# snphbaum/scikit-gpuppy

Hardware: NVIDIA B200
Metric: fit_s_per_iter (lower is better)
Workload: dtype f64

## Files before the change

### scikit-gpuppy_b200/csrc/gpk.cu

```cuda
#include "../../include/gpk.h"
#include "../../include/gpk_test.h"

#include <climits>
#include <new>
#include <vector>

#include "dgemm_dmma.cuh"
#include "factor.cuh"
#include "se_kernels.cuh"
#include "exact_kernels.cuh"
#include "periodic_kernels.cuh"

namespace gpk {
thread_local char g_err[512] = {0};
thread_local long g_launch_count = 0;
thread_local bool g_prof_on = false;
static thread_local std::vector<ProfPair> g_prof;
void prof_push(cudaEvent_t a, cudaEvent_t b) { g_prof.push_back(ProfPair{a, b}); }

struct Handle {
  int n = 0, d = 0, npad = 0;
  double *X = nullptr, *W = nullptr;
  bool own_X = false, own_W = false;
  double *x = nullptr, *xT = nullptr, *t = nullptr, *y = nullptr, *alpha = nullptr, *dL = nullptr;
  double* scal = nullptr;
  int* info = nullptr;
  double* part = nullptr; size_t part_elems = 0;
  double* G = nullptr; size_t G_elems = 0;
  double* colsq = nullptr; size_t colsq_elems = 0;
  double* pairdot = nullptr;
  double* dots = nullptr; size_t dots_elems = 0;
  long batch_rows = 0;
  SEHyper hyp;
  int kind = KIND_SE;
  double theta[3 * MAX_D + 2];
  bool factored = false, have_inverse = false;
  bool matrix_state = false;
  double logdet = 0.0, quad = 0.0, alpha2 = 0.0;
  cudaStream_t st = nullptr;
  cudaStream_t side = nullptr;
  std::vector<cudaEvent_t> events;
  int ev_next = 0;
  bool oz_want = false;
  bool oz_on = false;
  int oz_moduli_req = 0;
  size_t oz_out_cap = 0;
  oz::Workspace oz;
  oz::Workspace ozq;
  oz::Operand xs;
  bool x_sliced = false;
  cudaStream_t chain_st = nullptr;
  std::vector<cudaStream_t> ovl_st;
  std::vector<oz::Workspace> ovl_ws;
  cudaEvent_t ev_in = nullptr, ev_out = nullptr;
  bool ovl_on = false;
  double* raw_pinned = nullptr;
  bool grad_pending = false;
};

thread_local int g_overlap_T = 1;

static void release_overlap(Handle* h) {
  for (auto& w : h->ovl_ws) w.release();
  h->ovl_ws.clear();
  for (auto& s : h->ovl_st) if (s) { cudaStreamSynchronize(s); cudaStreamDestroy(s); }
  h->ovl_st.clear();
  if (h->chain_st) { cudaStreamSynchronize(h->chain_st); cudaStreamDestroy(h->chain_st); h->chain_st = nullptr; }
  if (h->ev_in) { cudaEventDestroy(h->ev_in); h->ev_in = nullptr; }
  if (h->ev_out) { cudaEventDestroy(h->ev_out); h->ev_out = nullptr; }
  h->ovl_on = false;
}

static int ensure_overlap(Handle* h) {
  if (h->ovl_on || !h->oz_on || !g_overlap_T) return 0;
  int depths = 0;
  size_t need = 0;
  for (long hh = h->npad / 2 / TILE * TILE; hh >= h->oz.min_dim; hh = hh / 2 / TILE * TILE) {
    need += (size_t)h->oz.S * (hh + TILE) * (3 * (hh + TILE) + round_up_l(hh + TILE, 256)) + 6 * hh * sizeof(double);
    ++depths;
  }
  if (depths == 0) return 0;
  size_t free_b = 0, total_b = 0;
  if (cudaMemGetInfo(&free_b, &total_b) != cudaSuccess) { cudaGetLastError(); return 0; }
  if (free_b < need + ((size_t)28 << 30)) return 0;
  int least = 0, greatest = 0;
  GPK_CUDA_OK(cudaDeviceGetStreamPriorityRange(&least, &greatest));
  GPK_CUDA_OK(cudaStreamCreateWithPriority(&h->chain_st, cudaStreamNonBlocking, greatest));
  GPK_CUDA_OK(cudaEventCreateWithFlags(&h->ev_in, cudaEventDisableTiming));
  GPK_CUDA_OK(cudaEventCreateWithFlags(&h->ev_out, cudaEventDisableTiming));
  h->ovl_st.assign(depths, nullptr);
// ... 40 lines not shown
    }
  }
  return 0;
}

static int ensure(double** p, size_t* have, size_t need) {
  if (*have >= need) return 0;
  if (*p) GPK_CUDA_OK(cudaFree(*p));
  *p = nullptr;
  *have = 0;
  GPK_CUDA_OK(cudaMalloc((void**)p, need * sizeof(double)));
  *have = need;
  return 0;
}

__global__ void __launch_bounds__(256) col_sum_kernel(const double* __restrict__ part, long nrows, int ncols,
                                                      double* __restrict__ out) {
  __shared__ double red[8];
  const int c = blockIdx.x;
  double s = 0.0;
  for (long r = threadIdx.x; r < nrows; r += 256) s += part[r * ncols + c];
  s = block_sum_256(s, red);
  if (threadIdx.x == 0) out[c] = s;
}

__global__ void set_int_kernel(int* p, int v) { *p = v; }
__global__ void __launch_bounds__(256) axpy_kernel(double* __restrict__ y, const double* __restrict__ x, int n, double a) {
  const int i = blockIdx.x * 256 + threadIdx.x;
  if (i < n) y[i] = fma(a, x[i], y[i]);
}

static int launch_se_tiles(const double* x1, int n1, const double* x2, int n2, int d, const SEHyper& hyp, double* out,
                           long ld, int rows_out, int cols_out, int add_noise, int pad_identity, int lower_only,
                           cudaStream_t st) {
  SETileArgs a;
  a.x1 = x1; a.n1 = n1; a.x2 = x2; a.n2 = n2; a.d = d;
  a.out = out; a.ld = ld; a.rows_out = rows_out; a.cols_out = cols_out;
  a.add_noise = add_noise; a.pad_identity = pad_identity; a.lower_only = lower_only;
  a.vec_ok = ((ld % 2) == 0 && (reinterpret_cast<uintptr_t>(out) % 16) == 0) ? 1 : 0;
  if (rows_out <= 0 || cols_out <= 0) return 0;
  if (hyp.kind == KIND_PERIODIC) {
    dim3 pgrid((cols_out + PER_T - 1) / PER_T, (rows_out + PER_T - 1) / PER_T);
    periodic_tile_kernel<<<pgrid, 256, 0, st>>>(a, hyp);
    GPK_LAUNCH_OK();
    return 0;
  }
  dim3 grid((cols_out + TILE - 1) / TILE, (rows_out + TILE - 1) / TILE);
  se_tile_kernel<<<grid, SE_THREADS, 0, st>>>(a, hyp);
  GPK_LAUNCH_OK();
  return 0;
}

static int solve_one(Handle* h, const double* b_pad, double* y, double* out) {
  const int npad = h->npad;
  trmv_lower_kernel<<<(npad + 7) / 8, 256, 0, h->st>>>(h->X, npad, npad, b_pad, y);
  GPK_LAUNCH_OK();
  const int nchunks = (npad + TRMVT_ROWS - 1) / TRMVT_ROWS;
  GPK_TRY(ensure(&h->part, &h->part_elems, (size_t)nchunks * npad));
  dim3 grid(npad / 128, nchunks);
  trmv_lower_T_partial_kernel<<<grid, 128, 0, h->st>>>(h->X, npad, npad, y, h->part);
  GPK_LAUNCH_OK();
  sum_chunks_kernel<<<(npad + 255) / 256, 256, 0, h->st>>>(h->part, nchunks, npad, npad, out, 1.0, 0.0);
  GPK_LAUNCH_OK();
  return 0;
}

template <int DP>
static int launch_trace(Handle* h, int d0, int trb, int tre, double* partial) {
  const int nt = h->npad / TILE;
  const size_t smem = (size_t)2 * h->d * (TILE + 2) * sizeof(double);
  GPK_CUDA_OK(cudaFuncSetAttribute(grad_trace_kernel<DP>, cudaFuncAttributeMaxDynamicSharedMemorySize, (int)smem));
  dim3 grid(nt, tre - trb);
  grad_trace_kernel<DP><<<grid, 256, smem, h->st>>>(h->W, h->npad, h->alpha, h->x, h->n, h->d, d0, h->hyp, trb, partial);
  GPK_LAUNCH_OK();
  return 0;
}

static int trace_sums(Handle* h, int trb, int tre, double* raw_host, double* async_dst = nullptr) {
  const int d = h->d;
  const int nt = h->npad / TILE;
  for (int k = 0; k <= (h->kind == KIND_PERIODIC ? 3 * d + 2 : d + 2); ++k) raw_host[k] = 0.0;
  if (tre <= trb) return 0;
  if (h->kind != KIND_PERIODIC) {
    const int r0 = trb * TILE, r1 = (tre * TILE < h->n) ? tre * TILE : h->n;
    diag_sum_kernel<<<1, 256, 0, h->st>>>(h->W, h->npad, h->alpha, r0, r1, h->scal + 4);
    GPK_LAUNCH_OK();
    GPK_CUDA_OK(cudaMemcpyAsync(async_dst ? async_dst : raw_host + d + 1, h->scal + 4, 2 * sizeof(double),
                                cudaMemcpyDeviceToHost, h->st));
  }
  if (h->kind == KIND_PERIODIC) {
    const int DPp = d <= 4 ? 4 : d <= 8 ? 8 : 16;
    const int nc = 3 * DPp + 2;
    const long nsl = (long)nt * (tre - trb);
    GPK_TRY(ensure(&h->part, &h->part_elems, (size_t)nsl * nc + nc));
    double* psums = h->part + (size_t)nsl * nc;
    dim3 pgrid(nt, tre - trb);
    if (DPp == 4) periodic_trace_kernel<4><<<pgrid, 256, 0, h->st>>>(h->W, h->npad, h->alpha, h->x, h->n, d, h->hyp, trb, h->part);
    else if (DPp == 8) periodic_trace_kernel<8><<<pgrid, 256, 0, h->st>>>(h->W, h->npad, h->alpha, h->x, h->n, d, h->hyp, trb, h->part);
    else periodic_trace_kernel<16><<<pgrid, 256, 0, h->st>>>(h->W, h->npad, h->alpha, h->x, h->n, d, h->hyp, trb, h->part);
    GPK_LAUNCH_OK();
    col_sum_kernel<<<nc, 256, 0, h->st>>>(h->part, nsl, nc, psums);
    GPK_LAUNCH_OK();
    double ph[50];
    GPK_CUDA_OK(cudaMemcpyAsync(ph, psums, nc * sizeof(double), cudaMemcpyDeviceToHost, h->st));
    GPK_CUDA_OK(cudaStreamSynchronize(h->st));
    raw_host[0] = ph[0];
    for (int k = 0; k < d; ++k) {
      raw_host[1 + k] = ph[1 + k];
      raw_host[1 + d + k] = ph[1 + DPp + k];
      raw_host[1 + 2 * d + k] = ph[1 + 2 * DPp + k];
    }
    raw_host[3 * d + 1] = ph[3 * DPp + 1];
    raw_host[3 * d + 2] = 0.0;
    return 0;
  }
  int DP = d <= 4 ? 4 : d <= 8 ? 8 : d <= 16 ? 16 : 32;
  const long nslots = (long)nt * (tre - trb);
  const int nchunks = (d + DP - 1) / DP;
  GPK_TRY(ensure(&h->part, &h->part_elems, (size_t)nslots * (DP + 1) + (size_t)nchunks * (DP + 1)));
  double* sums = h->part + (size_t)nslots * (DP + 1);
  double host[2 * 33];
  for (int d0 = 0, ch = 0; d0 < d; d0 += DP, ++ch) {
    switch (DP) {
      case 4: GPK_TRY(launch_trace<4>(h, d0, trb, tre, h->part)); break;
      case 8: GPK_TRY(launch_trace<8>(h, d0, trb, tre, h->part)); break;
      case 16: GPK_TRY(launch_trace<16>(h, d0, trb, tre, h->part)); break;
      default: GPK_TRY(launch_trace<32>(h, d0, trb, tre, h->part)); break;
    }
    col_sum_kernel<<<DP + 1, 256, 0, h->st>>>(h->part, nslots, DP + 1, sums + ch * (DP + 1));
    GPK_LAUNCH_OK();
    double* dst = async_dst ? async_dst + 4 + ch * (DP + 1) : host + ch * 33;
    GPK_CUDA_OK(cudaMemcpyAsync(dst, sums + ch * (DP + 1), (DP + 1) * sizeof(double), cudaMemcpyDeviceToHost, h->st));
  }
  if (async_dst) return 0;
  GPK_CUDA_OK(cudaStreamSynchronize(h->st));
  for (int d0 = 0, ch = 0; d0 < d; d0 += DP, ++ch) {
    if (d0 == 0) raw_host[0] = host[0];
    for (int k = 0; k < DP && d0 + k < d; ++k) raw_host[1 + d0 + k] = host[ch * 33 + 1 + k];
  }
  return 0;
}

static void trace_unpack(const Handle* h, const double* pinned, double* raw_host) {
  const int d = h->d;
  const int DP = d <= 4 ? 4 : d <= 8 ? 8 : d <= 16 ? 16 : 32;
  raw_host[d + 1] = pinned[0];
  raw_host[d + 2] = pinned[1];
  for (int d0 = 0, ch = 0; d0 < d; d0 += DP, ++ch) {
    const double* src = pinned + 4 + ch * (DP + 1);
    if (d0 == 0) raw_host[0] = src[0];
// ... 242 lines not shown
  cudaFree(hh->x); cudaFree(hh->xT); cudaFree(hh->t); cudaFree(hh->y); cudaFree(hh->alpha); cudaFree(hh->dL);
  cudaFree(hh->scal); cudaFree(hh->info);
  for (auto& e : hh->events) if (e) cudaEventDestroy(e);
  if (hh->side) { cudaStreamSynchronize(hh->side); cudaStreamDestroy(hh->side); }
  if (hh->part) cudaFree(hh->part);
  if (hh->G) cudaFree(hh->G);
  if (hh->colsq) cudaFree(hh->colsq);
  if (hh->dots) cudaFree(hh->dots);
  hh->oz.release();
  hh->ozq.release();
  release_overlap(hh);
  if (hh->raw_pinned) cudaFreeHost(hh->raw_pinned);
  delete hh;
  return 0;
}

int gpk_set_stream(gpk_handle h, void* stream) {
  H_OR_FAIL(h);
  hh->st = reinterpret_cast<cudaStream_t>(stream);
  return 0;
}

int gpk_set_kernel(gpk_handle h, int kind) {
  H_OR_FAIL(h);
  if (kind != KIND_SE && kind != KIND_PERIODIC) { snprintf(g_err, sizeof(g_err), "unknown kernel kind %d", kind); return -2; }
  if (kind == KIND_PERIODIC && hh->d > PER_MAX_D) {
    snprintf(g_err, sizeof(g_err), "the periodic covariance supports d <= %d", PER_MAX_D);
    return -2;
  }
  hh->kind = kind;
  hh->factored = false;
  hh->have_inverse = false;
  hh->x_sliced = false;
  return 0;
}

int gpk_kernel_matrix_periodic(const double* x1, int64_t n1, const double* x2, int64_t n2, int64_t d, const double* theta,
                               int noise_mode, double* out, int64_t ld, void* stream) {
  SEHyper hyp;
  GPK_TRY(set_hyper(hyp, theta, (int)d, KIND_PERIODIC));
  return launch_se_tiles(x1, (int)n1, x2, (int)n2, (int)d, hyp, out, ld, (int)n1, (int)n2, noise_mode, 0, 0,
                         reinterpret_cast<cudaStream_t>(stream));
}

int gpk_set_route(gpk_handle h, int int8, int64_t min_dim, int moduli, int64_t plane_cap_bytes) {
  H_OR_FAIL(h);
  if (int8 && (min_dim != 0 && (min_dim < 2 * TILE || min_dim % TILE))) {
    snprintf(g_err, sizeof(g_err), "gpk_set_route: min_dim must be 0 (default 2048) or a multiple of 128 >= 256");
    return -2;
  }
  if (int8 && moduli != 0 && (moduli < oz::CRT_MIN_MODULI || moduli > oz::CRT_MAX_MODULI)) {
    snprintf(g_err, sizeof(g_err), "gpk_set_route: moduli must be 0 (automatic) or in [%d, %d]", oz::CRT_MIN_MODULI,
             oz::CRT_MAX_MODULI);
    return -2;
  }
  if (int8 && hh->npad > 98304) {
    snprintf(g_err, sizeof(g_err), "gpk_set_route: exact int32 accumulation needs npad <= 98304");
    return -2;
  }
  GPK_CUDA_OK(cudaStreamSynchronize(hh->st));
  hh->oz.release();
  hh->ozq.release();
  release_overlap(hh);
  hh->oz_on = false;
  hh->x_sliced = false;
  hh->factored = false;
  hh->have_inverse = false;
  hh->oz.min_dim = (int8 && min_dim) ? (int)min_dim : 2048;
  hh->oz_moduli_req = int8 ? moduli : 0;
  hh->oz_out_cap = plane_cap_bytes > 0 ? (size_t)plane_cap_bytes : 0;
  hh->oz_want = int8 != 0 && hh->npad >= hh->oz.min_dim;
  return 0;
}

int gpk_get_route(gpk_handle h, int* out) {
  H_OR_FAIL(h);
  const int S = hh->oz_on ? hh->oz.S
                          : (hh->oz_moduli_req ? hh->oz_moduli_req : oz::crt_moduli_for(hh->npad, 54));
  out[0] = hh->oz_want ? 1 : 0;
  out[1] = hh->oz_want ? S : 0;
  out[2] = hh->oz.min_dim;
  out[3] = hh->oz_want ? oz::crt_bits(hh->npad, S) : 53;
  return 0;
}

int gpk_set_batch_rows(gpk_handle h, int64_t rows) {
  H_OR_FAIL(h);
  hh->batch_rows = rows < 0 ? 0 : rows;
  return 0;
}

int gpk_set_data(gpk_handle h, const double* x_dev, const double* t_dev) {
  H_OR_FAIL(h);
  GPK_CUDA_OK(cudaMemcpyAsync(hh->x, x_dev, (size_t)hh->n * hh->d * sizeof(double), cudaMemcpyDeviceToDevice, hh->st));
  GPK_CUDA_OK(cudaMemsetAsync(hh->t, 0, (size_t)hh->npad * sizeof(double), hh->st));
  GPK_CUDA_OK(cudaMemcpyAsync(hh->t, t_dev, (size_t)hh->n * sizeof(double), cudaMemcpyDeviceToDevice, hh->st));
  transpose_x_kernel<<<(hh->npad + 255) / 256, 256, 0, hh->st>>>(hh->x, hh->n, hh->d, hh->xT, hh->npad);
  GPK_LAUNCH_OK();
  hh->factored = false;
  hh->have_inverse = false;
  return 0;
}

int gpk_kernel_matrix(const double* x1, int64_t n1, const double* x2, int64_t n2, int64_t d, const double* theta,
                      int add_noise, double* out, int64_t ld, void* stream) {
  SEHyper hyp;
  GPK_TRY(set_hyper(hyp, theta, (int)d));
  return launch_se_tiles(x1, (int)n1, x2, (int)n2, (int)d, hyp, out, ld, (int)n1, (int)n2, add_noise, 0, 0,
                         reinterpret_cast<cudaStream_t>(stream));
}

static int factorize_W(Handle* hh) {
  const int n = hh->n, npad = hh->npad;
  set_int_kernel<<<1, 1, 0, hh->st>>>(hh->info, INT_MAX);
  GPK_LAUNCH_OK();
  FactorCtx c{hh->W, hh->X, (long)npad, hh->dL, hh->info, hh->st};
  hh->ev_next = 0;
  c.side = hh->side; c.ev = hh->events.data(); c.ev_next = &hh->ev_next;
  c.oz = hh->oz_on ? &hh->oz : nullptr;
  const bool ovl = hh->oz_on && hh->ovl_on && g_overlap_T;
  if (ovl) {
    GPK_CUDA_OK(cudaEventRecord(hh->ev_in, hh->st));
    GPK_CUDA_OK(cudaStreamWaitEvent(hh->chain_st, hh->ev_in, 0));
    c.st = hh->chain_st;
    c.ovl_ws = hh->ovl_ws.data(); c.ovl_st = hh->ovl_st.data(); c.ovl_depths = (int)hh->ovl_ws.size();
  }
  const int rc_rec = potrf_inv_node(c, 0, npad);
  if (rc_rec < 0) {
    cudaDeviceSynchronize();
    return rc_rec;
  }
  if (ovl) {
    GPK_CUDA_OK(cudaEventRecord(hh->ev_out, hh->chain_st));
    GPK_CUDA_OK(cudaStreamWaitEvent(hh->st, hh->ev_out, 0));
  }
  GPK_TRY(solve_one(hh, hh->t, hh->y, hh->alpha));
  nll_scalars_kernel<<<1, 256, 0, hh->st>>>(hh->dL, hh->y, hh->alpha, n, hh->scal);
  GPK_LAUNCH_OK();
  int info = 0;
  double sc[3];
  GPK_CUDA_OK(cudaMemcpyAsync(&info, hh->info, sizeof(int), cudaMemcpyDeviceToHost, hh->st));
  GPK_CUDA_OK(cudaMemcpyAsync(sc, hh->scal, 3 * sizeof(double), cudaMemcpyDeviceToHost, hh->st));
  GPK_CUDA_OK(cudaStreamSynchronize(hh->st));
  if (info != INT_MAX) {
    snprintf(g_err, sizeof(g_err), "leading minor %d of K is not positive definite", info);
    return info > 0 ? info : 1;
  }
  hh->logdet = sc[0]; hh->quad = sc[1]; hh->alpha2 = sc[2];
  return 0;
}

int gpk_factorize(gpk_handle h, const double* theta, int want_inverse) {
  H_OR_FAIL(h);
  if (!same_theta(hh, theta)) {
    hh->factored = false;
    hh->have_inverse = false;
    hh->x_sliced = false;
    hh->grad_pending = false;
    GPK_TRY(set_hyper(hh->hyp, theta, hh->d, hh->kind));
    GPK_TRY(ensure_route(hh));
    const int n = hh->n, npad = hh->npad;
    GPK_TRY(launch_se_tiles(hh->x, n, hh->x, n, hh->d, hh->hyp, hh->W, npad, npad, npad,
                            hh->kind == KIND_PERIODIC ? 2 : 1, 1, 1, hh->st));
    const int rc = factorize_W(hh);
    if (rc != 0) return rc;
    memcpy(hh->theta, theta, sizeof(double) * theta_len(hh->kind, hh->d));
    hh->factored = true;
    hh->matrix_state = false;
  }
  if (want_inverse) GPK_TRY(do_lauum(hh));
  return 0;
}

__global__ void __launch_bounds__(256) load_matrix_kernel(const double* __restrict__ K, long ldk, int n,
                                                          double* __restrict__ W, long ld, int npad) {
  const int c = blockIdx.x * 256 + threadIdx.x;
  const int r = blockIdx.y;
  if (c >= npad || (c >> 7) > (r >> 7)) return;
  W[(long)r * ld + c] = (r < n && c < n) ? K[(long)r * ldk + c] : (r == c ? 1.0 : 0.0);
}

int gpk_factorize_matrix(gpk_handle h, const double* K_dev, int64_t ldk, int want_inverse) {
  H_OR_FAIL(h);
  if (!K_dev || ldk < hh->n) { snprintf(g_err, sizeof(g_err), "gpk_factorize_matrix: bad matrix argument"); return -2; }
  hh->factored = false;
  hh->have_inverse = false;
  hh->x_sliced = false;
  GPK_TRY(ensure_route(hh));
  dim3 grid((hh->npad + 255) / 256, hh->npad);
  load_matrix_kernel<<<grid, 256, 0, hh->st>>>(K_dev, ldk, hh->n, hh->W, hh->npad, hh->npad);
  GPK_LAUNCH_OK();
  const int rc = factorize_W(hh);
  if (rc != 0) return rc;
  hh->factored = true;
  hh->matrix_state = true;
  if (want_inverse) GPK_TRY(do_lauum(hh));
  return 0;
}

int gpk_nll_matrix(gpk_handle h, double* nll) {
  H_OR_FAIL(h);
  if (!hh->factored) { snprintf(g_err, sizeof(g_err), "not factored"); return -2; }
  const double two_pi = 6.283185307179586476925286766559;
  *nll = 0.5 * hh->n * log(two_pi) + 0.5 * hh->logdet + 0.5 * hh->quad;
  return 0;
}

int gpk_logdet(gpk_handle h, double* out) {
  H_OR_FAIL(h);
  if (!hh->factored) { snprintf(g_err, sizeof(g_err), "not factored"); return -2; }
  *out = hh->logdet;
  return 0;
}

int gpk_grad_trace_partial(gpk_handle h, int64_t trb, int64_t tre, double* out) {
  H_OR_FAIL(h);
  if (!hh->factored || !hh->have_inverse || hh->matrix_state) { snprintf(g_err, sizeof(g_err), "inverse not available"); return -2; }
  if (hh->kind != KIND_SE) { snprintf(g_err, sizeof(g_err), "sharded trace: Gaussian covariance only"); return -2; }
  const int nt = hh->npad / TILE;
  if (trb < 0) trb = 0;
// ... 117 lines not shown
                            hh->kind == KIND_PERIODIC ? 2 : 0, 0, 0, hh->st));
    rows_dot_kernel<<<(unsigned)((mb + 7) / 8), 256, 0, hh->st>>>(hh->G, npad, (int)mb, npad, hh->alpha, Ka + r0);
    GPK_LAUNCH_OK();
  }
  if (hh->kind != KIND_PERIODIC) {
    axpy_kernel<<<(n + 255) / 256, 256, 0, hh->st>>>(Ka, hh->alpha, n, hh->hyp.vt);
    GPK_LAUNCH_OK();
  }
  residual_max_kernel<<<64, 256, 0, hh->st>>>(Ka, hh->t, hh->alpha, n, mx);
  GPK_LAUNCH_OK();
  unsigned long long bits[3];
  GPK_CUDA_OK(cudaMemcpyAsync(bits, mx, sizeof(bits), cudaMemcpyDeviceToHost, hh->st));
  GPK_CUDA_OK(cudaStreamSynchronize(hh->st));
  for (int i = 0; i < 3; ++i) memcpy(out_host + i, bits + i, sizeof(double));
  return 0;
}

int gpk_get_alpha(gpk_handle h, double* out) {
  H_OR_FAIL(h);
  if (!hh->factored) { snprintf(g_err, sizeof(g_err), "not factored"); return -2; }
  GPK_CUDA_OK(cudaMemcpyAsync(out, hh->alpha, (size_t)hh->n * sizeof(double), cudaMemcpyDeviceToDevice, hh->st));
  return 0;
}

int gpk_import_state(gpk_handle h, const double* theta, const double* alpha_dev, int have_inverse) {
  H_OR_FAIL(h);
  GPK_TRY(set_hyper(hh->hyp, theta, hh->d, hh->kind));
  memcpy(hh->theta, theta, sizeof(double) * theta_len(hh->kind, hh->d));
  GPK_CUDA_OK(cudaMemsetAsync(hh->alpha, 0, (size_t)hh->npad * sizeof(double), hh->st));
  GPK_CUDA_OK(cudaMemcpyAsync(hh->alpha, alpha_dev, (size_t)hh->n * sizeof(double), cudaMemcpyDeviceToDevice, hh->st));
  hh->factored = true;
  hh->matrix_state = false;
  hh->x_sliced = false;
  hh->have_inverse = have_inverse != 0;
  hh->logdet = NAN; hh->quad = NAN; hh->alpha2 = NAN;
  return 0;
}

int gpk_predict(gpk_handle h, const double* xs, int64_t m, double meant, double* mean, double* var, int want_var) {
  H_OR_FAIL(h);
  if (!hh->factored || hh->matrix_state) { snprintf(g_err, sizeof(g_err), "not factored from theta"); return -2; }
  if (m <= 0) return 0;
  const int npad = hh->npad, n = hh->n, d = hh->d;
  const long rows_max = batch_rows_for(hh, m);
  GPK_TRY(ensure_query_ws(hh, rows_max));
  const int nbi = npad / TILE;
  for (int64_t q0 = 0; q0 < m; q0 += rows_max) {
    const long mb = (m - q0) < rows_max ? (long)(m - q0) : rows_max;
    const long rows = round_up_l(mb, TILE);
    GPK_TRY(launch_se_tiles(xs + q0 * d, (int)mb, hh->x, n, d, hh->hyp, hh->G, npad, (int)rows, npad,
                            hh->kind == KIND_PERIODIC ? 2 : 0, 0, 0, hh->st));
    rows_dot_kernel<<<(unsigned)((mb + 7) / 8), 256, 0, hh->st>>>(hh->G, npad, (int)mb, npad, hh->alpha, mean + q0);
    GPK_LAUNCH_OK();
    if (meant != 0.0) {
      add_scalar_kernel<<<(unsigned)((mb + 255) / 256), 256, 0, hh->st>>>(mean + q0, (int)mb, meant);
      GPK_LAUNCH_OK();
    }
    if (want_var) {
      GPK_TRY(quad_forms(hh, rows));
      predict_var_kernel<<<(unsigned)((mb + 255) / 256), 256, 0, hh->st>>>(hh->colsq, rows, nbi, (int)mb,
                                                                            hh->hyp.v + hh->hyp.vt, var + q0);
      GPK_LAUNCH_OK();
    }
  }
  return 0;
}
// ... 242 lines not shown
  if (rc < 0) { cleanup(); return rc; }
  OZ_OK(cudaEventRecord(e1, st));
  if (reps < 1) reps = 1;
  for (int r = 0; r < reps && rc == 0; ++r) rc = oz::gemm_sliced(a, b, C, ldc, alpha, beta, krange, lower_only, st);
  if (rc < 0) { cleanup(); return rc; }
  OZ_OK(cudaEventRecord(e2, st));
  OZ_OK(cudaStreamSynchronize(st));
  if (ms_out) {
    OZ_OK(cudaEventElapsedTime(&ms_out[0], e0, e1));
    OZ_OK(cudaEventElapsedTime(&ms_out[1], e1, e2));
    ms_out[1] /= reps;
  }
#undef OZ_OK
  cleanup();
  return 0;
}

int gpk_test_tune(int group_m, int recon_cw) {
  if (group_m > 0) oz::g_group_m = group_m;
  if (recon_cw == 1 || recon_cw == 2 || recon_cw == 4) oz::g_recon_cw = recon_cw;
  return 0;
}

int gpk_test_position_lock(int on) {
  if (on >= 0 && on <= 2) oz::g_position_lock = on;
  return oz::g_position_lock;
}

int gpk_test_overlap(int on) {
  if (on == 0 || on == 1) g_overlap_T = on;
  return g_overlap_T;
}

int gpk_profile(int on) {
  g_prof_on = on != 0;
  return 0;
}

int gpk_profile_read(double* gemm_ms, int64_t* gemm_launches, int64_t* all_launches, double* max_gemm_ms) {
  double total = 0.0, longest = 0.0;
  for (auto& p : g_prof) {
    float ms = 0.f;
    cudaError_t e = cudaEventSynchronize(p.b);
    if (e == cudaSuccess) e = cudaEventElapsedTime(&ms, p.a, p.b);
    cudaEventDestroy(p.a);
    cudaEventDestroy(p.b);
    if (e != cudaSuccess) {
      snprintf(g_err, sizeof(g_err), "gpk_profile_read: %s", cudaGetErrorString(e));
      g_prof.clear();
      return -1;
    }
    total += ms;
    if (ms > longest) longest = ms;
  }
  if (max_gemm_ms) *max_gemm_ms = longest;
  if (gemm_ms) *gemm_ms = total;
  if (gemm_launches) *gemm_launches = (int64_t)g_prof.size();
  if (all_launches) *all_launches = (int64_t)g_launch_count;
  g_prof.clear();
  g_launch_count = 0;
  return 0;
}

int gpk_microbench_i8(int64_t iters, double seconds, double* out_host) {
  int nsm = 0, dev = 0;
  GPK_CUDA_OK(cudaGetDevice(&dev));
// ... 81 lines not shown
```

### scikit-gpuppy_b200/csrc/se_kernels.cuh

```cuda
#pragma once
#include "gpk_common.cuh"

namespace gpk {

constexpr int MAX_D = 64;
constexpr int SE_DCH = 16;

constexpr int KIND_SE = 0;
constexpr int KIND_PERIODIC = 1;

struct SEHyper {
  double v, vt;
  double w[MAX_D];
  double sw[MAX_D];
  int kind;
  double pf[16];
  double w2[16];
  double pr[16];
};

struct SETileArgs {
  const double* x1; int n1;
  const double* x2; int n2;
  int d;
  double* out; long ld;
  int rows_out, cols_out;
  int add_noise;
  int pad_identity;
  int lower_only;
  int vec_ok;
};

constexpr int SE_THREADS = 512;
__global__ void __launch_bounds__(SE_THREADS, 1) se_tile_kernel(SETileArgs p, SEHyper h) {
  const int bj = blockIdx.x, bi = blockIdx.y;
  if (p.lower_only && bj > bi) return;
  __shared__ __align__(16) double xa[SE_DCH][TILE];
  __shared__ __align__(16) double xb[SE_DCH][TILE];
  const int tid = threadIdx.x;
  const int tx = tid & 15, ty = (tid >> 4) & 15, tz = tid >> 8;
  const int row0 = bi * TILE, col0 = bj * TILE;

  double acc[4][8];
#pragma unroll
  for (int a = 0; a < 4; ++a)
#pragma unroll
    for (int b = 0; b < 8; ++b) acc[a][b] = 0.0;

  for (int k0 = 0; k0 < p.d; k0 += SE_DCH) {
    const int kc = min(SE_DCH, p.d - k0);
    __syncthreads();
    for (int idx = tid; idx < TILE * SE_DCH; idx += SE_THREADS) {
      const int r = idx / SE_DCH, k = idx % SE_DCH;
      double va = 0.0, vb = 0.0;
      if (k < kc) {
        const double s = h.sw[k0 + k];
        if (row0 + r < p.n1) va = p.x1[(long)(row0 + r) * p.d + k0 + k] * s;
        if (col0 + r < p.n2) vb = p.x2[(long)(col0 + r) * p.d + k0 + k] * s;
      }
      xa[k][r] = va;
      xb[k][r] = vb;
    }
    __syncthreads();
    for (int k = 0; k < kc; ++k) {
      double av[4];
      double2 bv[4];
#pragma unroll
      for (int a = 0; a < 4; ++a) av[a] = xa[k][ty + 16 * (a + 4 * tz)];
#pragma unroll
      for (int b = 0; b < 4; ++b) bv[b] = *reinterpret_cast<const double2*>(&xb[k][32 * b + 2 * tx]);
#pragma unroll
      for (int a = 0; a < 4; ++a)
#pragma unroll
        for (int b = 0; b < 4; ++b) {
          const double d0 = av[a] - bv[b].x, d1 = av[a] - bv[b].y;
          acc[a][2 * b] = fma(d0, d0, acc[a][2 * b]);
          acc[a][2 * b + 1] = fma(d1, d1, acc[a][2 * b + 1]);
        }
    }
  }

#pragma unroll
  for (int a = 0; a < 4; ++a) {
    const int row = row0 + ty + 16 * (a + 4 * tz);
    if (row >= p.rows_out) continue;
#pragma unroll
    for (int b = 0; b < 4; ++b) {
      const int col = col0 + 32 * b + 2 * tx;
      double o[2];
#pragma unroll
      for (int e = 0; e < 2; ++e) {
        const int c = col + e;
        double val;
        if (row < p.n1 && c < p.n2) {
          val = h.v * exp(-0.5 * acc[a][2 * b + e]);
          if (p.add_noise && row == c) val += h.vt;
        } else {
          val = (p.pad_identity && row == c) ? 1.0 : 0.0;
        }
        o[e] = val;
      }
      double* dst = p.out + (long)row * p.ld + col;
      if (p.vec_ok && col + 1 < p.cols_out) {
        *reinterpret_cast<double2*>(dst) = make_double2(o[0], o[1]);
      } else {
        if (col < p.cols_out) dst[0] = o[0];
        if (col + 1 < p.cols_out) dst[1] = o[1];
      }
    }
  }
}

template <int DP>
__global__ void __launch_bounds__(256, (DP <= 16) ? 2 : 1)
grad_trace_kernel(const double* __restrict__ Kinv, long ld, const double* __restrict__ alpha,
                  const double* __restrict__ x, int n, int d, int d0 , SEHyper h,
                  int tile_row_begin, double* __restrict__ partial ) {
  const int bj = blockIdx.x, bi = tile_row_begin + blockIdx.y;
  double* out = partial + ((long)blockIdx.y * gridDim.x + blockIdx.x) * (DP + 1);
  if (bj > bi) {
    if (threadIdx.x <= DP) out[threadIdx.x] = 0.0;
    return;
  }

  extern __shared__ __align__(16) double gsm[];
  constexpr int XLD = TILE + 2;
  constexpr int RT = 2;
  double* xa = gsm;
  double* xb = gsm + (long)d * XLD;
  __shared__ double al_a[TILE], al_b[TILE];
  __shared__ double red[8];
  const int tid = threadIdx.x;
  const int row0 = bi * TILE, col0 = bj * TILE;

  for (int idx = tid; idx < TILE * d; idx += 256) {
    const int r = idx / d, k = idx % d;
    xa[k * XLD + r] = (row0 + r < n) ? x[(long)(row0 + r) * d + k] : 0.0;
    xb[k * XLD + r] = (col0 + r < n) ? x[(long)(col0 + r) * d + k] : 0.0;
  }
  if (tid < TILE) {
    al_a[tid] = (row0 + tid < n) ? alpha[row0 + tid] : 0.0;
    al_b[tid] = (col0 + tid < n) ? alpha[col0 + tid] : 0.0;
  }
  __syncthreads();

  double g0 = 0.0;
  double gk[DP];
#pragma unroll
  for (int k = 0; k < DP; ++k) gk[k] = 0.0;

  const int c = tid & 127;
// ... 46 lines not shown
          sq[2 * i2][k] = d0v * d0v;
          sq[2 * i2 + 1][k] = d1v * d1v;
          dist[2 * i2] = fma(wk, sq[2 * i2][k], dist[2 * i2]);
          dist[2 * i2 + 1] = fma(wk, sq[2 * i2 + 1][k], dist[2 * i2 + 1]);
        }
      } else {
#pragma unroll
        for (int i = 0; i < RT; ++i) sq[i][k] = 0.0;
      }
    }
    for (int k = d0 + DP; k < d; ++k) {
      const double bv = xb[k * XLD + c];
#pragma unroll
      for (int i = 0; i < RT; ++i) {
        const double df = xa[k * XLD + r0 + i] - bv;
        dist[i] = fma(h.w[k] * df, df, dist[i]);
      }
    }
#pragma unroll
    for (int i = 0; i < RT; ++i) {
      const double pk = m[i] * h.v * exp(-0.5 * dist[i]);
      g0 += pk;
#pragma unroll
      for (int k = 0; k < DP; ++k) gk[k] = fma(pk, sq[i][k], gk[k]);
    }
  }

  double s = block_sum_256(g0, red);
  if (tid == 0) out[0] = s;
#pragma unroll
  for (int k = 0; k < DP; ++k) {
    s = block_sum_256(gk[k], red);
    if (tid == 0) out[1 + k] = s;
  }
}

__global__ void __launch_bounds__(256) diag_sum_kernel(const double* __restrict__ W, long ld,
                                                       const double* __restrict__ alpha, int r0, int r1,
                                                       double* __restrict__ out) {
  __shared__ double red[8];
  double s = 0.0, a2 = 0.0;
  for (int i = r0 + threadIdx.x; i < r1; i += 256) {
    s += W[(long)i * ld + i];
    a2 = fma(alpha[i], alpha[i], a2);
  }
  s = block_sum_256(s, red);
  a2 = block_sum_256(a2, red);
  if (threadIdx.x == 0) {
    out[0] = s;
    out[1] = a2;
  }
}

struct GAArgs {
  const double* xT; long ldxt;
  int n, npad, d, P;
  const double* U;
  const double* S;
  int sigma_full;
  double* G; long ldg;
  int rows_pad;
  int Q;
};

__global__ void __launch_bounds__(256) ga_build_kernel(GAArgs p, SEHyper h) {
  const int q = blockIdx.y;
// ... 121 lines not shown
```

### scikit-gpuppy_b200/skgpuppy/_native.py

```python
import ctypes
import os

import numpy as np

_HERE = os.path.dirname(os.path.abspath(__file__))
_LIB_PATH = os.path.join(_HERE, "libgpk.so")
_lib = None

c_double_p = ctypes.POINTER(ctypes.c_double)
c_int_p = ctypes.POINTER(ctypes.c_int)
i64 = ctypes.c_int64
vp = ctypes.c_void_p

SIGNATURES = {
    "gpk_version": (ctypes.c_int, []),
    "gpk_last_error": (ctypes.c_char_p, []),
    "gpk_npad": (i64, [i64]),
    "gpk_create": (ctypes.c_int, [i64, i64, vp, vp, ctypes.POINTER(vp)]),
    "gpk_destroy": (ctypes.c_int, [vp]),
    "gpk_set_stream": (ctypes.c_int, [vp, vp]),
    "gpk_set_data": (ctypes.c_int, [vp, vp, vp]),
    "gpk_kernel_matrix": (ctypes.c_int, [vp, i64, vp, i64, i64, c_double_p, ctypes.c_int, vp, i64, vp]),
    "gpk_factorize": (ctypes.c_int, [vp, c_double_p, ctypes.c_int]),
    "gpk_factorize_matrix": (ctypes.c_int, [vp, vp, i64, ctypes.c_int]),
    "gpk_nll_matrix": (ctypes.c_int, [vp, c_double_p]),
    "gpk_logdet": (ctypes.c_int, [vp, c_double_p]),
    "gpk_nll_grad": (ctypes.c_int, [vp, c_double_p, c_double_p, c_double_p, ctypes.c_int]),
    "gpk_grad_trace_partial": (ctypes.c_int, [vp, i64, i64, c_double_p]),
    "gpk_solve": (ctypes.c_int, [vp, vp, i64, vp]),
    "gpk_inverse": (ctypes.c_int, [vp, vp, i64]),
    "gpk_solve_residual": (ctypes.c_int, [vp, c_double_p]),
    "gpk_get_alpha": (ctypes.c_int, [vp, vp]),
    "gpk_import_state": (ctypes.c_int, [vp, c_double_p, vp, ctypes.c_int]),
    "gpk_predict": (ctypes.c_int, [vp, vp, i64, ctypes.c_double, vp, vp, ctypes.c_int]),
    "gpk_predict_cross": (ctypes.c_int, [vp, vp, i64, i64, vp, ctypes.c_double, vp, vp]),
    "gpk_propagate_ga": (ctypes.c_int, [vp, vp, vp, i64, ctypes.c_int, ctypes.c_double, vp, vp]),
    "gpk_propagate_ga_parts": (ctypes.c_int, [vp, vp, vp, i64, ctypes.c_int, vp, vp]),
    "gpk_propagate_exact": (ctypes.c_int, [vp, vp, vp, vp, vp, i64, ctypes.c_double, vp, vp]),
    "gpk_set_kernel": (ctypes.c_int, [vp, ctypes.c_int]),
    "gpk_kernel_matrix_periodic": (ctypes.c_int, [vp, i64, vp, i64, i64, c_double_p, ctypes.c_int, vp, i64, vp]),
    "gpk_set_route": (ctypes.c_int, [vp, ctypes.c_int, i64, ctypes.c_int, i64]),
    "gpk_get_route": (ctypes.c_int, [vp, c_int_p]),
    "gpk_set_batch_rows": (ctypes.c_int, [vp, i64]),
}

TEST_SIGNATURES = {
    "gpk_test_gemm": (ctypes.c_int, [ctypes.c_int, ctypes.c_int, ctypes.c_int, vp, i64, vp, i64, vp, i64, i64, i64,
                                     i64, ctypes.c_double, ctypes.c_double, ctypes.c_int, ctypes.c_int, vp, vp, i64,
                                     vp]),
    "gpk_test_potrf_inv": (ctypes.c_int, [vp, vp, i64, i64, vp, c_int_p, vp]),
    "gpk_test_lauum": (ctypes.c_int, [vp, vp, i64, i64, vp]),
    "gpk_test_oz_residues": (ctypes.c_int, [vp, i64, i64, i64, ctypes.c_int, ctypes.c_int, ctypes.c_int, vp, vp, vp]),
    "gpk_test_oz_gemm": (ctypes.c_int, [vp, i64, ctypes.c_int, ctypes.c_int, vp, i64, ctypes.c_int, ctypes.c_int, vp, i64,
                                        i64, i64, i64, ctypes.c_double, ctypes.c_double, ctypes.c_int, ctypes.c_int,
                                        ctypes.c_int, i64, ctypes.c_int, ctypes.POINTER(ctypes.c_float), vp]),
    "gpk_test_tune": (ctypes.c_int, [ctypes.c_int, ctypes.c_int]),
    "gpk_test_overlap": (ctypes.c_int, [ctypes.c_int]),
    "gpk_test_position_lock": (ctypes.c_int, [ctypes.c_int]),
    "gpk_profile": (ctypes.c_int, [ctypes.c_int]),
    "gpk_profile_read": (ctypes.c_int, [c_double_p, ctypes.POINTER(i64), ctypes.POINTER(i64), c_double_p]),
    "gpk_microbench": (ctypes.c_int, [ctypes.c_int, i64, c_double_p]),
    "gpk_microbench_i8": (ctypes.c_int, [i64, ctypes.c_double, c_double_p]),
}


class GpkError(RuntimeError):
    pass


def lib_path():
    return _LIB_PATH


def load():
    global _lib
    if _lib is not None:
        return _lib
    if not os.path.exists(_LIB_PATH):
        raise GpkError(
            "libgpk.so not found at %s: build it with `python scikit-gpuppy_b200/build_native.py` "
            "(there is no CPU fallback)" % _LIB_PATH)
    lib = ctypes.CDLL(_LIB_PATH)
    for name, (res, args) in list(SIGNATURES.items()) + list(TEST_SIGNATURES.items()):
        fn = getattr(lib, name)
        fn.restype = res
        fn.argtypes = args
    _lib = lib
    return lib


# ... 35 lines not shown
```

Before: 0.2906.

## Mirror SE kernel into upper triangle and read stored K in gradient trace

When building the squared-exponential K for large npad, the tile kernel also writes each lower tile, transposed through shared memory, into the upper triangle of W. The upper triangle then still holds K after the lower triangle is factored and inverted. The gradient trace kernel for off-diagonal tiles can then read the stored K values with a cp.async multi-stage pipeline instead of recomputing the exponentials. Diagonal tiles still use the recomputing kernel. This trades exp recomputation for extra strided global writes during matrix build and extra memory reads during the trace, and it assumes the inverse only overwrites the lower triangle.

```diff
diff --git a/scikit-gpuppy_b200/csrc/gpk.cu b/scikit-gpuppy_b200/csrc/gpk.cu
--- a/scikit-gpuppy_b200/csrc/gpk.cu
+++ b/scikit-gpuppy_b200/csrc/gpk.cu
@@ -56,6 +56,8 @@
   bool ovl_on = false;
   double* raw_pinned = nullptr;
   bool grad_pending = false;
+  bool knl_in_w = false;
+  bool trace_stored_ok = true;
 };
 
 thread_local int g_overlap_T = 1;
@@ -162,11 +164,16 @@
 
 static int launch_se_tiles(const double* x1, int n1, const double* x2, int n2, int d, const SEHyper& hyp, double* out,
                            long ld, int rows_out, int cols_out, int add_noise, int pad_identity, int lower_only,
-                           cudaStream_t st) {
+                           cudaStream_t st, int mirror = 0) {
   SETileArgs a;
   a.x1 = x1; a.n1 = n1; a.x2 = x2; a.n2 = n2; a.d = d;
   a.out = out; a.ld = ld; a.rows_out = rows_out; a.cols_out = cols_out;
   a.add_noise = add_noise; a.pad_identity = pad_identity; a.lower_only = lower_only;
+  a.mirror = mirror;
+  if (mirror && (x1 != x2 || n1 != n2 || rows_out != cols_out || hyp.kind != KIND_SE)) {
+    snprintf(g_err, sizeof(g_err), "launch_se_tiles: the mirror store needs the square Gaussian K");
+    return -2;
+  }
   a.vec_ok = ((ld % 2) == 0 && (reinterpret_cast<uintptr_t>(out) % 16) == 0) ? 1 : 0;
   if (rows_out <= 0 || cols_out <= 0) return 0;
   if (hyp.kind == KIND_PERIODIC) {
@@ -195,12 +202,27 @@
   return 0;
 }
 
+constexpr int TRACE_STORED_MIN_NPAD = 8192;
+
+static bool trace_reads_k(const Handle* h) { return h->knl_in_w && h->trace_stored_ok && h->kind == KIND_SE; }
+
 template <int DP>
 static int launch_trace(Handle* h, int d0, int trb, int tre, double* partial) {
   const int nt = h->npad / TILE;
   const size_t smem = (size_t)2 * h->d * (TILE + 2) * sizeof(double);
+  dim3 grid(nt, tre - trb);
+  if (trace_reads_k(h)) {
+    const size_t ssmem = grad_trace_stored_smem<DP>();
+    GPK_CUDA_OK(cudaFuncSetAttribute(grad_trace_stored_kernel<DP>, cudaFuncAttributeMaxDynamicSharedMemorySize, (int)ssmem));
+    grad_trace_stored_kernel<DP><<<grid, 256, ssmem, h->st>>>(h->W, h->npad, h->alpha, h->x, h->n, h->d, d0, trb, partial);
+    GPK_LAUNCH_OK();
+    GPK_CUDA_OK(cudaFuncSetAttribute(grad_trace_kernel<DP, true>, cudaFuncAttributeMaxDynamicSharedMemorySize, (int)smem));
+    grad_trace_kernel<DP, true><<<dim3(1, tre - trb), 256, smem, h->st>>>(h->W, h->npad, h->alpha, h->x, h->n, h->d, d0,
+                                                                          h->hyp, trb, partial + (size_t)nt * (tre - trb) * (DP + 1));
+    GPK_LAUNCH_OK();
+    return 0;
+  }
   GPK_CUDA_OK(cudaFuncSetAttribute(grad_trace_kernel<DP>, cudaFuncAttributeMaxDynamicSharedMemorySize, (int)smem));
-  dim3 grid(nt, tre - trb);
   grad_trace_kernel<DP><<<grid, 256, smem, h->st>>>(h->W, h->npad, h->alpha, h->x, h->n, h->d, d0, h->hyp, trb, partial);
   GPK_LAUNCH_OK();
   return 0;
@@ -245,7 +267,7 @@
     return 0;
   }
   int DP = d <= 4 ? 4 : d <= 8 ? 8 : d <= 16 ? 16 : 32;
-  const long nslots = (long)nt * (tre - trb);
+  const long nslots = (long)nt * (tre - trb) + (trace_reads_k(h) ? tre - trb : 0);
   const int nchunks = (d + DP - 1) / DP;
   GPK_TRY(ensure(&h->part, &h->part_elems, (size_t)nslots * (DP + 1) + (size_t)nchunks * (DP + 1)));
   double* sums = h->part + (size_t)nslots * (DP + 1);
@@ -554,6 +576,7 @@
   hh->factored = false;
   hh->have_inverse = false;
   hh->x_sliced = false;
+  hh->knl_in_w = false;
   return 0;
 }
 
@@ -588,6 +611,7 @@
   hh->x_sliced = false;
   hh->factored = false;
   hh->have_inverse = false;
+  hh->knl_in_w = false;
   hh->oz.min_dim = (int8 && min_dim) ? (int)min_dim : 2048;
   hh->oz_moduli_req = int8 ? moduli : 0;
   hh->oz_out_cap = plane_cap_bytes > 0 ? (size_t)plane_cap_bytes : 0;
@@ -621,6 +645,7 @@
   GPK_LAUNCH_OK();
   hh->factored = false;
   hh->have_inverse = false;
+  hh->knl_in_w = false;
   return 0;
 }
 
@@ -679,16 +704,19 @@
     hh->have_inverse = false;
     hh->x_sliced = false;
     hh->grad_pending = false;
+    hh->knl_in_w = false;
     GPK_TRY(set_hyper(hh->hyp, theta, hh->d, hh->kind));
     GPK_TRY(ensure_route(hh));
     const int n = hh->n, npad = hh->npad;
+    const bool mirror = hh->kind == KIND_SE && npad >= TRACE_STORED_MIN_NPAD;
     GPK_TRY(launch_se_tiles(hh->x, n, hh->x, n, hh->d, hh->hyp, hh->W, npad, npad, npad,
-                            hh->kind == KIND_PERIODIC ? 2 : 1, 1, 1, hh->st));
+                            hh->kind == KIND_PERIODIC ? 2 : 1, 1, 1, hh->st, mirror ? 1 : 0));
     const int rc = factorize_W(hh);
     if (rc != 0) return rc;
     memcpy(hh->theta, theta, sizeof(double) * theta_len(hh->kind, hh->d));
     hh->factored = true;
     hh->matrix_state = false;
+    hh->knl_in_w = mirror;
   }
   if (want_inverse) GPK_TRY(do_lauum(hh));
   return 0;
@@ -708,6 +736,7 @@
   hh->factored = false;
   hh->have_inverse = false;
   hh->x_sliced = false;
+  hh->knl_in_w = false;
   GPK_TRY(ensure_route(hh));
   dim3 grid((hh->npad + 255) / 256, hh->npad);
   load_matrix_kernel<<<grid, 256, 0, hh->st>>>(K_dev, ldk, hh->n, hh->W, hh->npad, hh->npad);
@@ -891,6 +920,7 @@
   hh->factored = true;
   hh->matrix_state = false;
   hh->x_sliced = false;
+  hh->knl_in_w = false;
   hh->have_inverse = have_inverse != 0;
   hh->logdet = NAN; hh->quad = NAN; hh->alpha2 = NAN;
   return 0;
@@ -1199,6 +1229,12 @@
   return g_overlap_T;
 }
 
+int gpk_test_trace_stored(void* h, int on) {
+  H_OR_FAIL(h);
+  if (on == 0 || on == 1) hh->trace_stored_ok = on == 1;
+  return trace_reads_k(hh) ? 1 : 0;
+}
+
 int gpk_profile(int on) {
   g_prof_on = on != 0;
   return 0;
diff --git a/scikit-gpuppy_b200/csrc/se_kernels.cuh b/scikit-gpuppy_b200/csrc/se_kernels.cuh
--- a/scikit-gpuppy_b200/csrc/se_kernels.cuh
+++ b/scikit-gpuppy_b200/csrc/se_kernels.cuh
@@ -1,5 +1,6 @@
 #pragma once
 #include "gpk_common.cuh"
+#include "dgemm_dmma.cuh"
 
 namespace gpk {
 
@@ -29,14 +30,19 @@
   int pad_identity;
   int lower_only;
   int vec_ok;
+  int mirror;
 };
 
 constexpr int SE_THREADS = 512;
+constexpr int SE_TLD = 33;
 __global__ void __launch_bounds__(SE_THREADS, 1) se_tile_kernel(SETileArgs p, SEHyper h) {
   const int bj = blockIdx.x, bi = blockIdx.y;
   if (p.lower_only && bj > bi) return;
-  __shared__ __align__(16) double xa[SE_DCH][TILE];
-  __shared__ __align__(16) double xb[SE_DCH][TILE];
+  __shared__ __align__(16) double sbuf[TILE * SE_TLD];
+  double (*xa)[TILE] = reinterpret_cast<double (*)[TILE]>(sbuf);
+  double (*xb)[TILE] = reinterpret_cast<double (*)[TILE]>(sbuf + SE_DCH * TILE);
+  double (*tr)[SE_TLD] = reinterpret_cast<double (*)[SE_TLD]>(sbuf);
+  static_assert(TILE * SE_TLD >= 2 * SE_DCH * TILE, "staging buffer holds xa and xb");
   const int tid = threadIdx.x;
   const int tx = tid & 15, ty = (tid >> 4) & 15, tz = tid >> 8;
   const int row0 = bi * TILE, col0 = bj * TILE;
@@ -80,10 +86,11 @@
     }
   }
 
+  const bool mirror = p.mirror && bi > bj;
 #pragma unroll
   for (int a = 0; a < 4; ++a) {
     const int row = row0 + ty + 16 * (a + 4 * tz);
-    if (row >= p.rows_out) continue;
+    if (mirror) __syncthreads();
 #pragma unroll
     for (int b = 0; b < 4; ++b) {
       const int col = col0 + 32 * b + 2 * tx;
@@ -100,23 +107,36 @@
         }
         o[e] = val;
       }
-      double* dst = p.out + (long)row * p.ld + col;
-      if (p.vec_ok && col + 1 < p.cols_out) {
-        *reinterpret_cast<double2*>(dst) = make_double2(o[0], o[1]);
-      } else {
-        if (col < p.cols_out) dst[0] = o[0];
-        if (col + 1 < p.cols_out) dst[1] = o[1];
-      }
-    }
-  }
-}
-
-template <int DP>
+      if (row < p.rows_out) {
+        double* dst = p.out + (long)row * p.ld + col;
+        if (p.vec_ok && col + 1 < p.cols_out) {
+          *reinterpret_cast<double2*>(dst) = make_double2(o[0], o[1]);
+        } else {
+          if (col < p.cols_out) dst[0] = o[0];
+          if (col + 1 < p.cols_out) dst[1] = o[1];
+        }
+      }
+      if (mirror) {
+        tr[32 * b + 2 * tx][ty + 16 * tz] = o[0];
+        tr[32 * b + 2 * tx + 1][ty + 16 * tz] = o[1];
+      }
+    }
+    if (mirror) {
+      __syncthreads();
+      const int j = tid & 31;
+      const int r = row0 + (j & 15) + 16 * a + 64 * (j >> 4);
+      for (int c = tid >> 5; c < TILE; c += SE_THREADS / 32)
+        if (col0 + c < p.rows_out && r < p.rows_out) p.out[(long)(col0 + c) * p.ld + r] = tr[c][j];
+    }
+  }
+}
+
+template <int DP, bool DIAG = false>
 __global__ void __launch_bounds__(256, (DP <= 16) ? 2 : 1)
 grad_trace_kernel(const double* __restrict__ Kinv, long ld, const double* __restrict__ alpha,
                   const double* __restrict__ x, int n, int d, int d0 , SEHyper h,
                   int tile_row_begin, double* __restrict__ partial ) {
-  const int bj = blockIdx.x, bi = tile_row_begin + blockIdx.y;
+  const int bi = tile_row_begin + blockIdx.y, bj = DIAG ? bi : (int)blockIdx.x;
   double* out = partial + ((long)blockIdx.y * gridDim.x + blockIdx.x) * (DP + 1);
   if (bj > bi) {
     if (threadIdx.x <= DP) out[threadIdx.x] = 0.0;
@@ -229,6 +249,127 @@
   for (int k = 0; k < DP; ++k) {
     s = block_sum_256(gk[k], red);
     if (tid == 0) out[1 + k] = s;
+  }
+}
+
+constexpr int GTS_ROWS = 8;
+constexpr int GTS_STAGES = 5;
+constexpr int GTS_LD = TILE + 2;
+constexpr int GTS_XLD = TILE + 2;
+template <int DP>
+constexpr size_t grad_trace_stored_smem() {
+  return sizeof(double) * ((size_t)DP * GTS_XLD + 2 * (size_t)GTS_STAGES * GTS_ROWS * GTS_LD);
+}
+
+__device__ __forceinline__ void cp_async8(double* dst, const double* src) {
+  asm volatile("cp.async.ca.shared.global [%0], [%1], 8;" ::"r"((uint32_t)__cvta_generic_to_shared(dst)), "l"(src)
+               : "memory");
+}
+
+template <int DP>
+__global__ void __launch_bounds__(256, (DP <= 16) ? 2 : 1)
+grad_trace_stored_kernel(const double* __restrict__ W, long ld, const double* __restrict__ alpha,
+                         const double* __restrict__ x, int n, int d, int d0, int tile_row_begin,
+                         double* __restrict__ partial ) {
+  const int bj = blockIdx.x, bi = tile_row_begin + blockIdx.y;
+  double* out = partial + ((long)blockIdx.y * gridDim.x + blockIdx.x) * (DP + 1);
+  if (bj >= bi) {
+    if (threadIdx.x <= DP) out[threadIdx.x] = 0.0;
+    return;
+  }
+  extern __shared__ __align__(16) double gsm[];
+  double* xa = gsm;
+  double* kin = xa + DP * GTS_XLD;
+  double* kst = kin + GTS_STAGES * GTS_ROWS * GTS_LD;
+  __shared__ double al_a[TILE];
+  __shared__ double red[8][DP + 1];
+  const int tid = threadIdx.x;
+  const int row0 = bi * TILE, col0 = bj * TILE;
+  const int dk = min(DP, d - d0);
+
+  auto issue = [&](int s) {
+    double* ki = kin + (s % GTS_STAGES) * GTS_ROWS * GTS_LD;
+    double* ks = kst + (s % GTS_STAGES) * GTS_ROWS * GTS_LD;
+    const int rs = row0 + s * GTS_ROWS;
+#pragma unroll
+    for (int j = 0; j < 2; ++j) {
+      const int idx = tid + 256 * j, r = idx >> 6, c2 = (idx & 63) * 2;
+      cp_async16(ki + r * GTS_LD + c2, W + (long)(rs + r) * ld + col0 + c2);
+    }
+#pragma unroll
+    for (int j = 0; j < 4; ++j) {
+      const int idx = tid + 256 * j, c = idx >> 3, r = idx & 7;
+      cp_async8(ks + r * GTS_LD + c, W + (long)(col0 + c) * ld + rs + r);
+    }
+  };
+  constexpr int NST = TILE / GTS_ROWS;
+#pragma unroll
+  for (int s = 0; s < GTS_STAGES - 1; ++s) {
+    issue(s);
+    cp_async_commit();
+  }
+
+  for (int idx = tid; idx < TILE * DP; idx += 256) {
+    const int r = idx / DP, k = idx % DP;
+    xa[k * GTS_XLD + r] = (k < dk && row0 + r < n) ? x[(long)(row0 + r) * d + d0 + k] : 0.0;
+  }
+  if (tid < TILE) al_a[tid] = (row0 + tid < n) ? alpha[row0 + tid] : 0.0;
+
+  const int c = tid & 127;
+  const int rq = (tid >> 7) * (GTS_ROWS / 2);
+  const bool col_ok = (col0 + c) < n;
+  const double alc = col_ok ? alpha[col0 + c] : 0.0;
+  double xb[DP];
+#pragma unroll
+  for (int k = 0; k < DP; ++k) xb[k] = (k < dk && col_ok) ? x[(long)(col0 + c) * d + d0 + k] : 0.0;
+  double g0 = 0.0;
+  double gk[DP];
+#pragma unroll
+  for (int k = 0; k < DP; ++k) gk[k] = 0.0;
+
+  for (int s = 0; s < NST; ++s) {
+    cp_async_wait<GTS_STAGES - 2>();
+    __syncthreads();
+    if (s + GTS_STAGES - 1 < NST) issue(s + GTS_STAGES - 1);
+    cp_async_commit();
+    const double* ki = kin + (s % GTS_STAGES) * GTS_ROWS * GTS_LD;
+    const double* ks = kst + (s % GTS_STAGES) * GTS_ROWS * GTS_LD;
+    const int r0 = s * GTS_ROWS + rq;
+#pragma unroll
+    for (int i2 = 0; i2 < GTS_ROWS / 4; ++i2) {
+      double pk[2];
+#pragma unroll
+      for (int e = 0; e < 2; ++e) {
+        const int i = 2 * i2 + e;
+        const bool ok = col_ok && (row0 + r0 + i) < n;
+        const double m = ok ? 2.0 * (ki[(rq + i) * GTS_LD + c] - al_a[r0 + i] * alc) : 0.0;
+        pk[e] = m * ks[(rq + i) * GTS_LD + c];
+        g0 += pk[e];
+      }
+#pragma unroll
+      for (int k = 0; k < DP; ++k) {
+        const double2 av = *reinterpret_cast<const double2*>(&xa[k * GTS_XLD + r0 + 2 * i2]);
+        const double e0 = av.x - xb[k], e1 = av.y - xb[k];
+        gk[k] = fma(pk[0] * e0, e0, gk[k]);
+        gk[k] = fma(pk[1] * e1, e1, gk[k]);
+      }
+    }
+  }
+
+  const int lane = tid & 31, warp = tid >> 5;
+  double v = warp_sum(g0);
+  if (lane == 0) red[warp][0] = v;
+#pragma unroll
+  for (int k = 0; k < DP; ++k) {
+    v = warp_sum(gk[k]);
+    if (lane == 0) red[warp][1 + k] = v;
+  }
+  __syncthreads();
+  if (tid <= DP) {
+    double sum = 0.0;
+#pragma unroll
+    for (int w = 0; w < 8; ++w) sum += red[w][tid];
+    out[tid] = sum;
   }
 }
 
diff --git a/scikit-gpuppy_b200/skgpuppy/_native.py b/scikit-gpuppy_b200/skgpuppy/_native.py
--- a/scikit-gpuppy_b200/skgpuppy/_native.py
+++ b/scikit-gpuppy_b200/skgpuppy/_native.py
@@ -56,6 +56,7 @@
                                         ctypes.c_int, i64, ctypes.c_int, ctypes.POINTER(ctypes.c_float), vp]),
     "gpk_test_tune": (ctypes.c_int, [ctypes.c_int, ctypes.c_int]),
     "gpk_test_overlap": (ctypes.c_int, [ctypes.c_int]),
+    "gpk_test_trace_stored": (ctypes.c_int, [vp, ctypes.c_int]),
     "gpk_test_position_lock": (ctypes.c_int, [ctypes.c_int]),
     "gpk_profile": (ctypes.c_int, [ctypes.c_int]),
     "gpk_profile_read": (ctypes.c_int, [c_double_p, ctypes.POINTER(i64), ctypes.POINTER(i64), c_double_p]),
```

Result: faster. 0.2877, median of 6 (-1.0%).
